# GuyTevet/motion-diffusion-model

Hardware: AMD Instinct MI355X
Metric: motions/sec (B=128, T=196, 50-step DDPM) (higher is better)
Workload: dtype f16x3 (fp32 operands split into fp16 hi+lo, 3 fp16 MFMA products, fp32 accumulate; everything else fp32); 1 GPU; HumanML3D text2motion, 50-step p_sample_loop with CFG 2.5 (2 denoiser forwards per step), batch=128 per GPU, T=196, 8-layer d=512 trans_enc MDM, random-init weights, cached text embedding; global_batch=128, diffusion_steps=50, parallelism=dp1: batch shards, no data-path collective, all_gather of final samples

## Files before the change

motion-diffusion-model_amd/csrc/common.h:

```cpp
#pragma once
#ifdef MDM_EMU
#include "hip_emu.h"
#else
#include <hip/hip_runtime.h>
#define MDM_DYN_SMEM(type, name) \
  extern __shared__ __attribute__((aligned(16))) unsigned char mdm_dyn_smem_raw[]; \
  type* name = reinterpret_cast<type*>(mdm_dyn_smem_raw)
#define MDM_LAUNCH(kernel, grid, block, shmem, stream, ...) \
  hipLaunchKernelGGL(kernel, (grid), (block), (shmem), (stream), __VA_ARGS__)
#endif
#include <stdint.h>
#include <type_traits>
#include <utility>

namespace mdm {

typedef float f32x16 __attribute__((ext_vector_type(16)));
typedef short p16x8 __attribute__((ext_vector_type(8)));

constexpr int kWave = 64;

constexpr int kMaxDevices = 64;
inline int rt_device_ordinal() {
#ifdef MDM_EMU
// ... 231 lines not shown
}

__device__ __forceinline__ void glds16(const void* gsrc_lane, void* lds_wave_base) {
#ifdef MDM_EMU
  emu::vm_issue(static_cast<char*>(lds_wave_base) + 16 * emu::lane_id(), gsrc_lane, 16, false);
#else
  __builtin_amdgcn_global_load_lds((const __attribute__((address_space(1))) void*)gsrc_lane,
                                   (__attribute__((address_space(3))) void*)lds_wave_base, 16, 0, 0);
#endif
}

__device__ __forceinline__ void glds16_nt(const void* gsrc_lane, void* lds_wave_base) {
#ifdef MDM_EMU
  emu::vm_issue(static_cast<char*>(lds_wave_base) + 16 * emu::lane_id(), gsrc_lane, 16, false);
#else
  __builtin_amdgcn_global_load_lds((const __attribute__((address_space(1))) void*)gsrc_lane,
                                   (__attribute__((address_space(3))) void*)lds_wave_base, 16, 0, 2);
#endif
}

template <class F, int... Is>
__device__ __forceinline__ void static_for_impl(F&& f, std::integer_sequence<int, Is...>) {
  (f(std::integral_constant<int, Is>{}), ...);
}
template <int N, class F>
__device__ __forceinline__ void static_for(F&& f) {
  static_for_impl(f, std::make_integer_sequence<int, N>{});
}

#ifdef MDM_EMU
__device__ __forceinline__ void lds_read16(p16x8& dst, const unsigned char* base, uint32_t byte_off) {
  emu::lds_issue(&dst, base + byte_off, 16);
}
template <int N> __device__ __forceinline__ void lds_wait(p16x8&, p16x8&) { emu::lgkm_wait(N); }
template <int N> __device__ __forceinline__ void lds_wait(p16x8&, p16x8&, p16x8&, p16x8&) { emu::lgkm_wait(N); }
template <int N> __device__ __forceinline__ void lds_wait(p16x8&, p16x8&, p16x8&, p16x8&, p16x8&, p16x8&) { emu::lgkm_wait(N); }
template <int N>
__device__ __forceinline__ void lds_wait(p16x8&, p16x8&, p16x8&, p16x8&, p16x8&, p16x8&, p16x8&, p16x8&) { emu::lgkm_wait(N); }
#else
template <int IMM> __device__ __forceinline__ void lds_read16(p16x8& dst, uint32_t lds_addr) {
  asm volatile("ds_read_b128 %0, %1 offset:%2" : "=v"(dst) : "v"(lds_addr), "i"(IMM));
}
template <int N> __device__ __forceinline__ void lds_wait(p16x8& a, p16x8& b) {
  asm volatile("s_waitcnt lgkmcnt(%2)" : "+v"(a), "+v"(b) : "i"(N));
}
template <int N> __device__ __forceinline__ void lds_wait(p16x8& a, p16x8& b, p16x8& c, p16x8& d) {
  asm volatile("s_waitcnt lgkmcnt(%4)" : "+v"(a), "+v"(b), "+v"(c), "+v"(d) : "i"(N));
}
template <int N>
__device__ __forceinline__ void lds_wait(p16x8& a, p16x8& b, p16x8& c, p16x8& d, p16x8& e, p16x8& f, p16x8& g,
                                         p16x8& h) {
  asm volatile("s_waitcnt lgkmcnt(%8)"
               : "+v"(a), "+v"(b), "+v"(c), "+v"(d), "+v"(e), "+v"(f), "+v"(g), "+v"(h)
               : "i"(N));
}
template <int N>
__device__ __forceinline__ void lds_wait(p16x8& a, p16x8& b, p16x8& c, p16x8& d, p16x8& e, p16x8& f) {
  asm volatile("s_waitcnt lgkmcnt(%6)" : "+v"(a), "+v"(b), "+v"(c), "+v"(d), "+v"(e), "+v"(f) : "i"(N));
}
__device__ __forceinline__ uint32_t lds_addr_of(const void* p) {
  return (uint32_t)(uintptr_t)(const __attribute__((address_space(3))) void*)p;
}
#endif

#ifdef MDM_EMU
__device__ __forceinline__ void gload16_async(f32x4& dst, const float* p) { emu::vm_issue(&dst, p, 16, true); }
template <int N> __device__ __forceinline__ void vmem_wait(f32x4&, f32x4&, f32x4&, f32x4&) { emu::vm_wait(N); }
__device__ __forceinline__ void gload16_async(p16x8& dst, const p16_t* p) { emu::vm_issue(&dst, p, 16, true); }
__device__ __forceinline__ void gload16_refill(p16x8& slot, const p16_t* p) { emu::vm_issue(&slot, p, 16, true); }
template <int N> __device__ __forceinline__ void vmem_wait(p16x8&, p16x8&) { emu::vm_wait(N); }
template <int N> __device__ __forceinline__ void vmem_wait(p16x8&, p16x8&, p16x8&, p16x8&) { emu::vm_wait(N); }
template <int N> __device__ __forceinline__ void vmem_wait(p16x8&, p16x8&, p16x8&, p16x8&, p16x8&, p16x8&) { emu::vm_wait(N); }
template <int N>
__device__ __forceinline__ void vmem_wait(p16x8&, p16x8&, p16x8&, p16x8&, p16x8&, p16x8&, p16x8&, p16x8&) { emu::vm_wait(N); }
// ... 197 lines not shown
```

motion-diffusion-model_amd/csrc/gemm_x3.h:

```cpp
#pragma once
#include "attention_x3.h"
#include "common.h"
#include "gemm_f32.h"
#include <cstdlib>

namespace mdm {

constexpr int X3_TM = 224, X3_BK = 32;
constexpr int x3_tn(int waves) { return 32 * waves; }
constexpr int X3_MSUB = X3_TM / 32;
constexpr int X3_A_BYTES = X3_TM * X3_BK * 2;
constexpr int X3_A_STAGE = 2 * X3_A_BYTES;
constexpr int X3_A_RING = 2;
constexpr int X3_PIPE_RING = 4;
#ifndef MDM_X3_EPI_AHEAD
#define MDM_X3_EPI_AHEAD 0
#endif
constexpr bool X3_EPI_AHEAD = MDM_X3_EPI_AHEAD != 0;
#ifdef MDM_X3_PIPE_BADWAIT
constexpr int X3P_MID_SLACK = 8;
#else
constexpr int X3P_MID_SLACK = 0;
#endif
#if defined(MDM_X3_PIPE_WDRAIN)
constexpr int X3P_WAIT_WS = 0, X3P_WAIT_MID = 0;
#elif defined(MDM_X3_PIPE_STRICT)
constexpr int X3P_WAIT_WS = 6, X3P_WAIT_MID = 3;
#else
constexpr int X3P_WAIT_WS = 12, X3P_WAIT_MID = 7;
#endif
constexpr int x3_patch_base(int ring) { return ring * X3_A_STAGE; }
constexpr int X3_PATCH_BYTES = 8 * 32 * 4;
constexpr int X3_TAB_BYTES = X3_TM * 8;
constexpr int x3_tab_base(int waves, int ring = X3_A_RING) { return x3_patch_base(ring) + waves * X3_PATCH_BYTES; }
constexpr int X3_RAW_BYTES = 7 * 1024;
constexpr int x3_raw_base(int waves, int ring = X3_A_RING) { return x3_tab_base(waves, ring) + 2 * X3_TAB_BYTES; }
constexpr int x3_part_base(int waves, int ring = X3_A_RING) { return x3_raw_base(waves, ring) + 2 * X3_RAW_BYTES; }
constexpr int X3_CVEC_BYTES = 4 * 1024;
constexpr int x3_cvec_base(int waves, bool ln, int ring = X3_A_RING) {
  return ln ? x3_part_base(waves, ring) + waves * X3_TAB_BYTES : x3_tab_base(waves, ring);
}
constexpr int x3_lds_bytes(int waves, bool ln, int ring = X3_A_RING) {
  return x3_cvec_base(waves, ln, ring) + 2 * X3_CVEC_BYTES;
}
constexpr int X3_A_GROUPS = X3_A_STAGE / 1024;
constexpr int x3_a_pieces(int waves) { return (X3_A_GROUPS + waves - 1) / waves; }

struct X3Operand {
  const p16_t* hi;
  const p16_t* lo;
};
struct X3Weights {
  const p16_t* hi;
  const p16_t* lo;
};
inline size_t x3_packed_weight_elems(int N, int K) { return (size_t)((N + 31) / 32 * 32) * K; }

struct X3Epilogue {
  float* out;
  const float* bias;
  const float* res;
  const p16_t* resh;
// ... 59 lines not shown
        const float back = p16_to_f32((p16_t)h8[j]);
        bad = bad || !(fabsf(back) <= 3.0e38f);
      }
      if (bad) *overflow = 1;
    }
    const int kstep = k8 >> 1, half = k8 & 1, lane = (n & 31) + 32 * half;
    const size_t o = (((size_t)(n >> 5) * (K / 16) + kstep) * 64 + lane) * 8;
    *reinterpret_cast<p16x8*>(hi + o) = h8;
    *reinterpret_cast<p16x8*>(lo + o) = l8;
  }
}

constexpr int x3_res_rounds(int t, bool t16) { return (t16 && t == X3_MSUB - 1) ? 2 : 4; }
constexpr int x3_res_younger_rounds(int t, int rr, bool t16) {
  int n = 0;
  for (int q = t + 1; q <= t + rr - 1 && q < X3_MSUB; ++q) n += x3_res_rounds(q, t16);
  return n;
}

#if !defined(MDM_EMU) && defined(MDM_PROBES)
#define MDM_X3_DBG 1
__device__ unsigned long long g_x3_dbg[8];
__device__ __forceinline__ unsigned long long x3_now() { return __builtin_readcyclecounter(); }
#endif

template <int PIECES>
struct X3Cursor {
  int v;
  int k;
  uint32_t off[PIECES];
};

template <int WAVES, int ACT, int RES, bool OUT_F32, bool OUT_PLANES, bool OUT_QKV, int ABL, bool FOLD = false,
          bool OSTAT = false, bool EMBED = false, bool T16 = false, bool F6 = false, bool PIPE = false, int NCB = 1>
__global__ __launch_bounds__(64 * WAVES, NCB == 2 ? 1 : 2) void gemm_x3_kernel(X3Operand A, X3Weights W, X3Epilogue ep, int M, int N,
                                                                     int K, int rows_per_tile, int tiles_n, int total) {
  MDM_DYN_SMEM(unsigned char, lds);
  static_assert(!PIPE || (T16 && (WAVES == 8 || (WAVES == 4 && NCB == 2)) && !F6), "the pipelined k-loop exists for 208-row (T16), 256-column tiles");
  static_assert(NCB == 1 || (NCB == 2 && PIPE && WAVES == 4), "two column blocks per wave: the pipelined 4-wave form only");
  constexpr int RINGN = PIPE ? X3_PIPE_RING : X3_A_RING;
  constexpr int NBLK = WAVES * NCB;
  constexpr int X3_WAVES = WAVES, X3_TN = 32 * NBLK, X3_A_PIECES = x3_a_pieces(WAVES);
  constexpr int NT32 = T16 ? X3_MSUB - 1 : X3_MSUB;
  constexpr int NROUNDS = 4 * NT32 + (T16 ? 2 : 0);
  using Cursor = X3Cursor<X3_A_PIECES>;

  const int tid = threadIdx.x;
  const int lane = tid & 63;
#ifdef MDM_EMU
  const int wid = tid >> 6;
#else
  const int wid = __builtin_amdgcn_readfirstlane(tid >> 6);
#endif
  const int r = lane & 31, h = lane >> 5;
  const int nk = K / X3_BK;
  const int gstride = (int)gridDim.x;

  auto tile_origin = [&](int v, int& m0, int& n0) {
    const int lid = xcd_remap(v, total);
    const int tile_m = lid / tiles_n, tile_n = lid - tile_m * tiles_n;
    m0 = tile_m * rows_per_tile;
    n0 = tile_n * X3_TN;
  };

  const int schunk = (lane & 3) ^ ((lane >> 4) & 3);
  auto aim_a = [&](Cursor& c) {
    int m0, n0;
    tile_origin(c.v, m0, n0);
#pragma unroll
    for (int i = 0; i < X3_A_PIECES; ++i) {
      const int jj = min(wid + X3_WAVES * i, 25);
      const int q = PIPE ? (jj < 13 ? jj : jj + 1) : min(wid + X3_WAVES * i, X3_A_GROUPS - 1);
// ... 61 lines not shown
  auto stats_dma = [&](int m0s, int par) {
    const float* st = FOLD ? ep.astat : ep.rstat;
    const int npieces = (X3_TM * ep.stat_parts * 8 + 1023) / 1024;
    for (int pc = wid; pc < npieces; pc += X3_WAVES) {
      const long long total_f = (long long)M * ep.stat_parts * 2;
      long long fo = (long long)m0s * ep.stat_parts * 2 + 4LL * (64 * pc + lane);
      if (fo >= total_f) fo = 0;
      glds16(st + fo, lds + x3_raw_base(NBLK, RINGN) + par * X3_RAW_BYTES + pc * 1024);
    }
  };
  constexpr bool LN_ANY = FOLD || OSTAT || RES == 3;
  auto cvec_dma = [&](int n0c, int par) {
    const float* src = nullptr;
    if (wid == 0) src = ep.bias;
    if constexpr (FOLD) { if (wid == 1) src = ep.colsum; }
    if constexpr (RES == 3) { if (wid == 2) src = ep.rgamma; if (wid == 3) src = ep.rbeta; }
    if (src != nullptr) glds16(src + min(n0c + 4 * lane, N - 4), lds + x3_cvec_base(NBLK, LN_ANY, RINGN) + par * X3_CVEC_BYTES + wid * 1024);
  };
  {
    int m0f, n0f;
    tile_origin(v, m0f, n0f);
    if constexpr (FOLD || RES == 3) stats_dma(m0f, 0);
    cvec_dma(n0f, 0);
  }
  p16x8 wh[2], wl[2], wnh[2], wnl[2];
  p16x8 wsh[4 * NCB] = {}, wsl[4 * NCB] = {};
  uint32_t wso = 0;
  uint32_t wtile = 0;
  auto aim_w_tile = [&]() {
    int m0w, n0w;
    tile_origin(wv, m0w, n0w);
    wtile = (uint32_t)((n0w >> 5) + wid * NCB) * (uint32_t)wk16 * 512u;
  };
  auto aim_w = [&]() { wso = wtile + (uint32_t)wkk * 1024u + (uint32_t)lane * 8u; };
  auto advance_w = [&]() {
    if (++wkk == nk) {
      wkk = 0;
      if (wv + gstride < total) { wv += gstride; aim_w_tile(); }
    }
  };
  auto load_w_half = [&](int ks, auto q_tag) __attribute__((always_inline)) {
    constexpr int q = decltype(q_tag)::value;
#pragma unroll
    for (int cb = 0; cb < NCB; ++cb) {
      const uint32_t o = wso + (uint32_t)cb * (uint32_t)wk16 * 512u + 512u * (uint32_t)ks;
#ifdef MDM_X3_PIPE_NOGUARD
      gload16_async(wsh[q * NCB + cb], W.hi + o);
      gload16_async(wsl[q * NCB + cb], W.lo + o);
#else
      gload16_refill(wsh[q * NCB + cb], W.hi + o);
      gload16_refill(wsl[q * NCB + cb], W.lo + o);
#endif
    }
  };
  auto wait_slot = [&](auto n_tag, auto q_tag) __attribute__((always_inline)) {
    constexpr int n = decltype(n_tag)::value, q = decltype(q_tag)::value;
    if constexpr (NCB == 1) vmem_wait<n>(wsh[q], wsl[q]);
    else vmem_wait<n>(wsh[2 * q], wsl[2 * q], wsh[2 * q + 1], wsl[2 * q + 1]);
  };
  auto wait_all_slots = [&]() __attribute__((always_inline)) {
    static_for<NCB>([&](auto c_tag) __attribute__((always_inline)) {
      constexpr int c4 = 4 * decltype(c_tag)::value;
      vmem_wait<0>(wsh[c4], wsl[c4], wsh[c4 + 1], wsl[c4 + 1], wsh[c4 + 2], wsl[c4 + 2], wsh[c4 + 3], wsl[c4 + 3]);
    });
  };
  int gs = 0;
#if defined(MDM_X3_PIPE_PRIO) && !defined(MDM_EMU)
  if constexpr (PIPE) { if (wid >= 4) __builtin_amdgcn_s_setprio(1); }
#endif
  if constexpr (PIPE) {
#pragma unroll
    for (int st = 0; st < 3; ++st) {
#pragma unroll
      for (int i = 0; i < X3_A_PIECES; ++i) piece_a(ca, i, st);
      advance_a(ca);
    }
    aim_w_tile();
#pragma unroll
    for (int st = 0; st < 2; ++st) {
      aim_w();
      if (st == 0) { load_w_half(0, std::integral_constant<int, 0>{}); load_w_half(1, std::integral_constant<int, 1>{}); }
      else { load_w_half(0, std::integral_constant<int, 2>{}); load_w_half(1, std::integral_constant<int, 3>{}); }
      advance_w();
    }
    wait_all_slots();
    wg_barrier();
  } else {
#pragma unroll
    for (int i = 0; i < X3_A_PIECES; ++i) piece_a(ca, i, 0);
    advance_a(ca);
    load_w(wv, wkk, wh, wl);
    wait_vmem_all();
    wg_barrier();
  }

  int abuf = 0;
  int tile_parity = 0;
  for (; v < total; v += gstride, tile_parity ^= 1) {
    int m0, n0;
    tile_origin(v, m0, n0);
    f32x16 accs_[NCB][NT32];
    f32x4 acc16s_[NCB][2];
#pragma unroll
    for (int cb = 0; cb < NCB; ++cb) {
#pragma unroll
      for (int t = 0; t < NT32; ++t)
#pragma unroll
        for (int e = 0; e < 16; ++e) accs_[cb][t][e] = 0.f;
      acc16s_[cb][0] = f32x4{0.f, 0.f, 0.f, 0.f};
      acc16s_[cb][1] = f32x4{0.f, 0.f, 0.f, 0.f};
    }
    f32x16 (&acc)[NT32] = accs_[0];
    f32x4 (&acc16)[2] = acc16s_[0];
    const int ncol0_w = n0 + wid * NCB * 32;
    const float* const cvec = reinterpret_cast<const float*>(lds + x3_cvec_base(NBLK, LN_ANY, RINGN) + tile_parity * X3_CVEC_BYTES);
    const int kt_cvec = nk > 1 ? 1 : 0;
    if (nk == 1) wg_barrier();
    constexpr bool LN_TABS = FOLD || RES == 3;
    float2* const stab = reinterpret_cast<float2*>(lds + x3_tab_base(NBLK, RINGN) + tile_parity * X3_TAB_BYTES);
    if constexpr (LN_TABS) {
      if (tid < X3_TM) {
        int m0t, n0t;
        tile_origin(v, m0t, n0t);
        const bool pad_row = m0t + tid >= M;
        const float* sraw = reinterpret_cast<const float*>(lds + x3_raw_base(NBLK, RINGN) + tile_parity * X3_RAW_BYTES);
        float s1 = 0.f;
        for (int p = 0; p < ep.stat_parts; ++p) s1 += sraw[(tid * ep.stat_parts + p) * 2];
        const float mean = s1 * ep.inv_dim;
        const float pcols = (float)ep.stat_cols, inv_pcols = 1.0f / pcols;
        float m2 = 0.f;
        for (int p = 0; p < ep.stat_parts; ++p) {
          const float dm = sraw[(tid * ep.stat_parts + p) * 2] * inv_pcols - mean;
          m2 += sraw[(tid * ep.stat_parts + p) * 2 + 1] + pcols * dm * dm;
        }
        const float var = m2 * ep.inv_dim;
#ifdef MDM_EMU
        stab[tid] = pad_row ? make_float2(0.f, 0.f) : make_float2(mean, 1.0f / sqrtf(var + 1e-5f));
#else
        stab[tid] = pad_row ? make_float2(0.f, 0.f) : make_float2(mean, __builtin_amdgcn_rsqf(var + 1e-5f));
#endif
      }
      if (v + gstride < total) {
        int m0n, n0n;
        tile_origin(v + gstride, m0n, n0n);
        stats_dma(m0n, tile_parity ^ 1);
      }
    }
    float2* const atab = stab;
    float2* const rtab = stab;
#ifdef MDM_X3_DBG
    unsigned long long dbg_t0 = 0, dbg_w0 = 0, dbg_w1 = 0, dbg_bar = 0;
    if constexpr ((ABL & 128) != 0) dbg_t0 = x3_now();
#endif
    if constexpr (PIPE) {
#ifndef MDM_X3_PIPE_DEPTH
#define MDM_X3_PIPE_DEPTH 2
#endif
      constexpr int NU = 2 * NT32, NE = NU + 1, XP = NT32, DEPTH = MDM_X3_PIPE_DEPTH, RING = DEPTH + 1;
      constexpr int LWH = 2 * NCB, NA_MIN = 26 / X3_WAVES;
      constexpr int WAIT_WS = (NCB == 1 && X3_WAVES == 8) ? X3P_WAIT_WS : 2 * NA_MIN + 3 * LWH;
      constexpr int WAIT_MID = (NCB == 1 && X3_WAVES == 8) ? X3P_WAIT_MID : NA_MIN + 2 * LWH;
      static_assert((NCB == 1 && X3_WAVES == 8) || (WAIT_WS == 24 && WAIT_MID == 14), "wide form: 4 waves x 2 column blocks");
      static_assert(NU % RING == 0, "fragment ring slots must line up across steps");
      p16x8 ah[RING], al[RING], a16h, a16l;
#ifndef MDM_EMU
      const uint32_t lane_a = lds_base + fa, lane_a16 = lds_base + fa16;
      const uint32_t sw0 = (uint32_t)((h ^ sw) * 16), sw1 = (uint32_t)(((2 + h) ^ sw) * 16);
#endif
      auto issue_reads = [&](auto ee_tag, uint32_t stg) __attribute__((always_inline)) {
        constexpr int ee = decltype(ee_tag)::value;
        if constexpr (ee == XP) {
#ifdef MDM_EMU
          lds_read16(a16h, lds + stg * X3_A_STAGE, fa16);
          lds_read16(a16l, lds + stg * X3_A_STAGE, X3_A_BYTES + fa16);
#else
          lds_read16<0>(a16h, lane_a16 + stg * X3_A_STAGE);
          lds_read16<X3_A_BYTES>(a16l, lane_a16 + stg * X3_A_STAGE);
#endif
        } else {
          constexpr int u = ee < XP ? ee : ee - 1, ks = u / NT32, t = u - ks * NT32;
#ifdef MDM_EMU
          lds_read16(ah[u % RING], lds + stg * X3_A_STAGE, fa + t * 2048 + (((ks * 2 + h) ^ sw) * 16));
          lds_read16(al[u % RING], lds + stg * X3_A_STAGE, X3_A_BYTES + fa + t * 2048 + (((ks * 2 + h) ^ sw) * 16));
#else
          const uint32_t ad = lane_a + stg * X3_A_STAGE + (ks ? sw1 : sw0);
          lds_read16<t * 2048>(ah[u % RING], ad);
          lds_read16<X3_A_BYTES + t * 2048>(al[u % RING], ad);
// ... 275 lines not shown
    constexpr bool COL_SCALE = x3_has_col_scale(ACT, RES);
    const float mult4 = (COL_SCALE && n4 < ep.scale_cols) ? ep.col_scale : 1.f;
    float4 c4 = zero4(), g4 = zero4(), be4 = zero4();
    if constexpr (FOLD) c4 = ld4(cvec + 256 + cl4);
    if constexpr (RES == 3) {
      g4 = ld4(cvec + 512 + cl4);
      be4 = ld4(cvec + 768 + cl4);
    }
    const float bias = cvec[wblk * 32 + r];
    float csum = 0.f;
    if constexpr (FOLD) csum = cvec[256 + wblk * 32 + r];
    const float accs = ep.acc_scale;
    const float4 bb4 = RES == 3 ? make_float4(b4.x + be4.x, b4.y + be4.y, b4.z + be4.z, b4.w + be4.w) : b4;
    auto finish4 = [&](float4 v4, float2 st) __attribute__((always_inline)) {
      v4.x *= accs; v4.y *= accs; v4.z *= accs; v4.w *= accs;
      if constexpr (FOLD) {
        v4.x = st.y * (v4.x - st.x * c4.x) + bb4.x; v4.y = st.y * (v4.y - st.x * c4.y) + bb4.y;
        v4.z = st.y * (v4.z - st.x * c4.z) + bb4.z; v4.w = st.y * (v4.w - st.x * c4.w) + bb4.w;
      } else {
        v4.x += bb4.x; v4.y += bb4.y; v4.z += bb4.z; v4.w += bb4.w;
      }
      if (ACT == ACT_GELU) { v4.x = gelu_erf_fast(v4.x); v4.y = gelu_erf_fast(v4.y); v4.z = gelu_erf_fast(v4.z); v4.w = gelu_erf_fast(v4.w); }
      else if (ACT == ACT_SILU) { v4.x = silu(v4.x); v4.y = silu(v4.y); v4.z = silu(v4.z); v4.w = silu(v4.w); }
      if constexpr (COL_SCALE) { v4.x *= mult4; v4.y *= mult4; v4.z *= mult4; v4.w *= mult4; }
      return v4;
    };
    auto row_stats = [&](auto j_tag) __attribute__((always_inline)) {
      constexpr int j = decltype(j_tag)::value;
      if constexpr (LN_TABS && j < NROUNDS) return stab[(j / 4) * 32 + 8 * (j % 4) + prow];
      else return make_float2(0.f, 1.f);
    };
    auto patch_write = [&](auto j_tag) __attribute__((always_inline)) {
      constexpr int j = decltype(j_tag)::value, t = j / 4, g = j % 4;
      if constexpr (j < 4 * NT32) {
#pragma unroll
        for (int e = 0; e < 4; ++e) patch[((e + 4 * h) << 5) + r] = acc[t][4 * g + e];
      } else if constexpr (T16 && j < NROUNDS) {
        if (h == g) {
#pragma unroll
          for (int cb = 0; cb < 2; ++cb)
#pragma unroll
            for (int e = 0; e < 4; ++e) patch[((e + 4 * (g16 & 1)) << 5) + 16 * cb + r16] = acc16[cb][e];
        }
      }
    };

    if (OUT_QKV) {
      const int Dm = ep.D, SPq = ep.qkv.SP, Hq = ep.qkv.H;
      int ncol_e = ncol0, m0_e = m0;
#ifndef MDM_EMU
      asm volatile("" : "+s"(ncol_e), "+s"(m0_e));
#endif
      const int which = ncol_e / Dm, hcol = ncol_e - which * Dm, head = hcol >> 7, d0 = hcol & 127;
      const size_t shq = (size_t)(m0_e / rows_per_tile) * Hq + head;
      if (ncol0 < N && !(ABL & 1)) {
        if (which == 2) {
          p16_t* vhp = ep.qkv.vh + ((shq * ep.qkv.NKT) * AX_HD + d0 + r) * 32 + 8 * h;
          p16_t* vlp = ep.qkv.vl + ((shq * ep.qkv.NKT) * AX_HD + d0 + r) * 32 + 8 * h;
          const int nkt = ep.qkv.NKT;
#pragma unroll
          for (int t = 0; t < NT32; ++t) {
            if (t < nkt) {
#pragma unroll
              for (int s2 = 0; s2 < 2; ++s2) {
                float vv[8];
#pragma unroll
                for (int j = 0; j < 8; ++j) {
                  if constexpr (FOLD) {
                    const float2 st = atab[32 * t + mfma_row(8 * s2 + j, h)];
                    vv[j] = st.y * (acc[t][8 * s2 + j] * accs - st.x * csum) + bias;
                  } else {
                    vv[j] = acc[t][8 * s2 + j] * accs + bias;
                  }
                }
                p16x8 vh8, vl8;
                split8(vv, vh8, vl8);
                *reinterpret_cast<p16x8*>(vhp + t * (AX_HD * 32) + 16 * s2) = vh8;
                *reinterpret_cast<p16x8*>(vlp + t * (AX_HD * 32) + 16 * s2) = vl8;
              }
            }
          }
          if constexpr (T16) {
            if (NT32 < nkt) {
#pragma unroll
              for (int cb = 0; cb < 2; ++cb) {
                const int cl = 16 * cb + r16;
                const float b16 = lane_bcast(bias, cl);
                const float c16 = FOLD ? lane_bcast(csum, cl) : 0.f;
                float vv[4];
#pragma unroll
                for (int e = 0; e < 4; ++e) {
                  if constexpr (FOLD) {
                    const float2 st = atab[192 + 4 * g16 + e];
                    vv[e] = st.y * (acc16[cb][e] * accs - st.x * c16) + b16;
                  } else {
                    vv[e] = acc16[cb][e] * accs + b16;
                  }
                }
                const size_t o = ((shq * ep.qkv.NKT + NT32) * AX_HD + d0 + cl) * 32 + 4 * ((g16 >> 1) + 2 * (g16 & 1));
                split4_store(ep.qkv.vh + o, ep.qkv.vl + o, make_float4(vv[0], vv[1], vv[2], vv[3]));
              }
            }
          }
        } else {
          p16_t* dh = (which == 0 ? ep.qkv.qh : ep.qkv.kh) + shq * SPq * AX_HD + d0 + pc4;
          p16_t* dl = (which == 0 ? ep.qkv.ql : ep.qkv.kl) + shq * SPq * AX_HD + d0 + pc4;
          const int nkt = ep.qkv.NKT;
          patch_write(std::integral_constant<int, 0>{});
          float2 st_cur = row_stats(std::integral_constant<int, 0>{});
          float4 v_cur = zero4();
          if constexpr (X3_EPI_AHEAD) {
            wave_lds_fence();
            v_cur = ld4(&patch[prow * 32 + pc4]);
            wave_lds_fence();
            patch_write(std::integral_constant<int, 1>{});
          }
          static_for<NROUNDS>([&](auto j_tag) __attribute__((always_inline)) {
            constexpr int j = decltype(j_tag)::value, t = j / 4, g = j % 4;
            float4 v4;
            float2 st_next;
            if constexpr (X3_EPI_AHEAD) {
              wave_lds_fence();
              float4 v_next = zero4();
              if constexpr (j + 1 < NROUNDS) v_next = ld4(&patch[prow * 32 + pc4]);
              st_next = row_stats(std::integral_constant<int, j + 1>{});
              wave_lds_fence();
              patch_write(std::integral_constant<int, j + 2>{});
              v4 = v_cur;
              v_cur = v_next;
            } else {
              wave_lds_fence();
              v4 = ld4(&patch[prow * 32 + pc4]);
              st_next = row_stats(std::integral_constant<int, j + 1>{});
              wave_lds_fence();
              patch_write(std::integral_constant<int, j + 1>{});
// ... 209 lines not shown
  (void)per_cu;
  return 3;
#else
  static int cus_of[kMaxDevices] = {};
  const int dev = rt_device_ordinal();
  int& cus = cus_of[dev];
  if (cus == 0) {
    hipDeviceProp_t prop;
    if (hipGetDeviceProperties(&prop, dev) == hipSuccess) cus = prop.multiProcessorCount;
    if (cus <= 0) cus = 256;
  }
  int wgs = per_cu * cus / 8 * 8;
#ifdef MDM_PROBES
  static const int div = [] { const char* e = getenv("MDM_X3_GRID_DIV"); return e != nullptr && atoi(e) > 1 ? atoi(e) : 1; }();
  wgs = wgs / div / 8 * 8;
#endif
  return wgs > 0 ? wgs : 8;
#endif
}

#ifdef MDM_PROBES
inline int& x3_waves_setting() {
  static int waves = [] {
    const char* e = getenv("MDM_X3_WAVES");
    return (e != nullptr && e[0] == '4') ? 4 : 8;
  }();
  return waves;
}
#else
inline int x3_waves_setting() { return 8; }
#endif

template <int WAVES, int ACT, int RES, bool OUT_F32, bool OUT_PLANES, bool OUT_QKV, int ABL, bool FOLD = false,
          bool OSTAT = false, bool EMBED = false, bool T16 = false, bool F6 = false, bool PIPE = false, int NCB = 1>
inline int launch_gemm_x3_w(const X3Operand& A, const X3Weights& W, const X3Epilogue& ep, int M, int N, int K,
                                int rpt, hipStream_t stream) {
  constexpr int NBLK = WAVES * NCB;
  constexpr int TN = 32 * NBLK;
  constexpr bool LN = FOLD || OSTAT || RES == 3;
  constexpr int RINGN = PIPE ? X3_PIPE_RING : X3_A_RING;
  const int tiles_m = (M + rpt - 1) / rpt, tiles_n = (N + TN - 1) / TN;
  const int total = tiles_m * tiles_n;
  static_assert(!(F6 && T16), "the f16f6 k-loop has no 16-row sub-tile yet");
  auto kfn = &gemm_x3_kernel<WAVES, ACT, RES, OUT_F32, OUT_PLANES, OUT_QKV, ABL, FOLD, OSTAT, EMBED, T16, F6, PIPE, NCB>;
  if (T16 && rpt > X3_TM - 16) return -2;
  if (PIPE && (K / X3_BK) % 2 != 0) return -2;
  if (!x3_has_col_scale(ACT, RES) && ep.scale_cols > 0) return -2;
#ifndef MDM_EMU
  if (x3_lds_bytes(NBLK, LN, RINGN) > 65536) {
    static bool configured[kMaxDevices] = {};
    if (const int rc = rt_dyn_lds_once(kfn, x3_lds_bytes(NBLK, LN, RINGN), configured, stream)) return rc;
  }
#endif
  const int grid = std::min(total, x3_grid_limit((WAVES == 4 && NCB == 1) ? 2 : 1));
  MDM_LAUNCH(kfn, dim3(grid), dim3(64 * WAVES), x3_lds_bytes(NBLK, LN, RINGN), stream, A, W, ep, M, N, K, rpt, tiles_n, total);
  return 0;
}

inline bool x3_wide_setting() {
#ifdef MDM_PROBES
  const char* e = getenv("MDM_X3_WIDE");
  return e != nullptr && e[0] == '1';
#else
  return false;
#endif
}

inline bool x3_pipe_setting(int kind = 0) {
#ifndef MDM_PROBES
  (void)kind;
  return true;
#else
  static const bool on = [] {
    const char* e = getenv("MDM_X3_PIPE");
    return !(e != nullptr && e[0] == '0');
  }();
  static const int kinds = [] {
    const char* e = getenv("MDM_X3_PIPE_KINDS");
    return e != nullptr ? atoi(e) : 0x3f;
  }();
  return on && ((kinds >> kind) & 1);
#endif
}

template <bool T16, bool PIPE = false, bool WIDE = false>
inline int launch_gemm_x3_ln_t(int kind, const X3Operand& A, const X3Weights& W, const X3Epilogue& ep, int M, int N,
                                   int K, int rpt, hipStream_t s) {
#ifdef MDM_PROBES
  if constexpr (WIDE) {
    switch (kind) {
      case 0: return launch_gemm_x3_w<4, ACT_NONE, 0, false, false, true, 0, true, false, false, T16, false, PIPE, 2>(A, W, ep, M, N, K, rpt, s);
      case 1: return launch_gemm_x3_w<4, ACT_NONE, 2, false, true, false, 0, false, true, false, T16, false, PIPE, 2>(A, W, ep, M, N, K, rpt, s);
      case 2: return launch_gemm_x3_w<4, ACT_NONE, 3, false, true, false, 0, false, true, false, T16, false, PIPE, 2>(A, W, ep, M, N, K, rpt, s);
      case 3: return launch_gemm_x3_w<4, ACT_GELU, 0, false, true, false, 0, true, false, false, T16, false, PIPE, 2>(A, W, ep, M, N, K, rpt, s);
      case 4: return launch_gemm_x3_w<4, ACT_NONE, 0, true, false, false, 0, true, false, false, T16, false, PIPE, 2>(A, W, ep, M, N, K, rpt, s);
      default: return -2;
    }
  }
#endif
  switch (kind) {
    case 0: return launch_gemm_x3_w<8, ACT_NONE, 0, false, false, true, 0, true, false, false, T16, false, PIPE>(A, W, ep, M, N, K, rpt, s);
    case 1: return launch_gemm_x3_w<8, ACT_NONE, 2, false, true, false, 0, false, true, false, T16, false, PIPE>(A, W, ep, M, N, K, rpt, s);
    case 2: return launch_gemm_x3_w<8, ACT_NONE, 3, false, true, false, 0, false, true, false, T16, false, PIPE>(A, W, ep, M, N, K, rpt, s);
    case 3: return launch_gemm_x3_w<8, ACT_GELU, 0, false, true, false, 0, true, false, false, T16, false, PIPE>(A, W, ep, M, N, K, rpt, s);
    case 4: return launch_gemm_x3_w<8, ACT_NONE, 0, true, false, false, 0, true, false, false, T16, false, PIPE>(A, W, ep, M, N, K, rpt, s);
    case 5:
      return launch_gemm_x3_w<8, ACT_NONE, 1, false, true, false, 0, false, false, true, T16>(A, W, ep, M, N, K, rpt, s);
    default: return -2;
  }
}
inline bool x3_t16_setting() {
#ifdef MDM_PROBES
  static const bool on = [] {
    const char* e = getenv("MDM_X3_T16");
    return !(e != nullptr && e[0] == '0');
  }();
  return on;
#else
  return true;
#endif
}
inline int launch_gemm_x3_ln(int kind, const X3Operand& A, const X3Weights& W, const X3Epilogue& ep, int M, int N,
                                 int K, int rpt, hipStream_t s) {
  if (rpt <= X3_TM - 16 && x3_t16_setting()) {
    if (kind != 5 && (K / X3_BK) % 2 == 0 && x3_pipe_setting(kind)) {
      if (x3_wide_setting()) return launch_gemm_x3_ln_t<true, true, true>(kind, A, W, ep, M, N, K, rpt, s);
      return launch_gemm_x3_ln_t<true, true>(kind, A, W, ep, M, N, K, rpt, s);
    }
    return launch_gemm_x3_ln_t<true>(kind, A, W, ep, M, N, K, rpt, s);
  }
  return launch_gemm_x3_ln_t<false>(kind, A, W, ep, M, N, K, rpt, s);
}

#ifdef MDM_PROBES
inline int& x3_pipe_probe() { static int on = 0; return on; }
#endif

template <int ACT, int RES, bool OUT_F32, bool OUT_PLANES, bool OUT_QKV, int ABL = 0>
inline int launch_gemm_x3_t(const X3Operand& A, const X3Weights& W, const X3Epilogue& ep, int M, int N, int K,
                                int rpt, hipStream_t stream) {
#ifdef MDM_PROBES
  if (x3_waves_setting() == 4)
    return launch_gemm_x3_w<4, ACT, RES, OUT_F32, OUT_PLANES, OUT_QKV, ABL>(A, W, ep, M, N, K, rpt, stream);
#endif
  return launch_gemm_x3_w<8, ACT, RES, OUT_F32, OUT_PLANES, OUT_QKV, ABL>(A, W, ep, M, N, K, rpt, stream);
}

inline int launch_gemm_x3(const X3Operand& A, const X3Weights& W, const X3Epilogue& ep, int M, int N, int K, int act,
                              int seq_len, hipStream_t s, int ablate = 0) {
  const bool res = ep.res != nullptr, f32 = ep.out != nullptr, pl = ep.oh != nullptr;
  const int rpt = x3_rows_per_tile(M, seq_len);
  if (ep.resh != nullptr) {
    if (ablate == 0 && act == ACT_NONE && !res && f32 && !pl)
      return launch_gemm_x3_t<ACT_NONE, 2, true, false, false>(A, W, ep, M, N, K, rpt, s);
    return -2;
  }
#ifdef MDM_PROBES
  if (x3_pipe_probe() != 0 && act == ACT_NONE && !res && f32 && !pl && M % 197 == 0 && (K / X3_BK) % 2 == 0) {
#define X3_PIPE_PROBE_CASE(c) case c: return x3_pipe_probe() == 1 \
      ? launch_gemm_x3_w<8, ACT_NONE, 0, true, false, false, c, false, false, false, true, false, true>(A, W, ep, M, N, K, 197, s) \
// ... 33 lines not shown
  if (act == ACT_NONE && res && f32 && !pl) return launch_gemm_x3_t<ACT_NONE, 1, true, false, false>(A, W, ep, M, N, K, rpt, s);
  if (act == ACT_GELU && !res && !f32 && pl) return launch_gemm_x3_t<ACT_GELU, 0, false, true, false>(A, W, ep, M, N, K, rpt, s);
  if (act == ACT_GELU && !res && f32 && !pl) return launch_gemm_x3_t<ACT_GELU, 0, true, false, false>(A, W, ep, M, N, K, rpt, s);
  if (act == ACT_GELU && res && f32 && !pl) return launch_gemm_x3_t<ACT_GELU, 1, true, false, false>(A, W, ep, M, N, K, rpt, s);
  if (act == ACT_SILU && !res && f32 && !pl) return launch_gemm_x3_t<ACT_SILU, 0, true, false, false>(A, W, ep, M, N, K, rpt, s);
  return -2;
}

#ifdef MDM_PROBES
inline int launch_gemm_f16f6(const X3Operand& A, const X3Weights& W, const X3Epilogue& ep, int M, int N, int K, int act,
                             hipStream_t s) {
  const bool res = ep.res != nullptr;
  if (act == ACT_NONE && !res && x3_waves_setting() == 4)
    return launch_gemm_x3_w<4, ACT_NONE, 0, true, false, false, 0, false, false, false, false, true>(A, W, ep, M, N, K, X3_TM, s);
  if (act == ACT_NONE && !res)
    return launch_gemm_x3_w<8, ACT_NONE, 0, true, false, false, 0, false, false, false, false, true>(A, W, ep, M, N, K, X3_TM, s);
  if (act == ACT_NONE && res)
    return launch_gemm_x3_w<8, ACT_NONE, 1, true, false, false, 0, false, false, false, false, true>(A, W, ep, M, N, K, X3_TM, s);
  if (act == ACT_GELU && !res)
    return launch_gemm_x3_w<8, ACT_GELU, 0, true, false, false, 0, false, false, false, false, true>(A, W, ep, M, N, K, X3_TM, s);
  return -2;
}
#endif

inline int launch_gemm_x3_qkv(const X3Operand& A, const X3Weights& W, const X3Epilogue& ep, int nseq, int S, int D,
                                  hipStream_t s) {
  if (S > X3_TM) return -2;
  if (x3_waves_setting() == 8 && S <= X3_TM - 16 && x3_t16_setting()) {
    if ((D / X3_BK) % 2 == 0 && x3_pipe_setting(5)) {
#ifdef MDM_PROBES
      if (x3_wide_setting())
        return launch_gemm_x3_w<4, ACT_NONE, 0, false, false, true, 0, false, false, false, true, false, true, 2>(A, W, ep, nseq * S,
                                                                                                                   3 * D, D, S, s);
#endif
      return launch_gemm_x3_w<8, ACT_NONE, 0, false, false, true, 0, false, false, false, true, false, true>(A, W, ep, nseq * S,
                                                                                                              3 * D, D, S, s);
    }
    return launch_gemm_x3_w<8, ACT_NONE, 0, false, false, true, 0, false, false, false, true>(A, W, ep, nseq * S, 3 * D, D,
                                                                                                 S, s);
  }
  return launch_gemm_x3_t<ACT_NONE, 0, false, false, true>(A, W, ep, nseq * S, 3 * D, D, S, s);
}

#endif

}
```

Measured before the change: 365.4 motions/s.

## Use 16x16x32 MFMA tiling in the pipelined x3 GEMM k-loop

Measured after the change: 396.3 motions/s (median of 6 runs). +8.5%, better.

```diff
diff --git a/motion-diffusion-model_amd/csrc/common.h b/motion-diffusion-model_amd/csrc/common.h
--- a/motion-diffusion-model_amd/csrc/common.h
+++ b/motion-diffusion-model_amd/csrc/common.h
@@ -287,6 +287,9 @@
 __device__ __forceinline__ void lds_read16(p16x8& dst, const unsigned char* base, uint32_t byte_off) {
   emu::lds_issue(&dst, base + byte_off, 16);
 }
+__device__ __forceinline__ void lds_refill16(p16x8& slot, const unsigned char* base, uint32_t byte_off) {
+  emu::lds_issue(&slot, base + byte_off, 16);
+}
 template <int N> __device__ __forceinline__ void lds_wait(p16x8&, p16x8&) { emu::lgkm_wait(N); }
 template <int N> __device__ __forceinline__ void lds_wait(p16x8&, p16x8&, p16x8&, p16x8&) { emu::lgkm_wait(N); }
 template <int N> __device__ __forceinline__ void lds_wait(p16x8&, p16x8&, p16x8&, p16x8&, p16x8&, p16x8&) { emu::lgkm_wait(N); }
@@ -295,6 +298,9 @@
 #else
 template <int IMM> __device__ __forceinline__ void lds_read16(p16x8& dst, uint32_t lds_addr) {
   asm volatile("ds_read_b128 %0, %1 offset:%2" : "=v"(dst) : "v"(lds_addr), "i"(IMM));
+}
+template <int IMM> __device__ __forceinline__ void lds_refill16(p16x8& slot, uint32_t lds_addr) {
+  asm volatile("ds_read_b128 %0, %1 offset:%2" : "+v"(slot) : "v"(lds_addr), "i"(IMM));
 }
 template <int N> __device__ __forceinline__ void lds_wait(p16x8& a, p16x8& b) {
   asm volatile("s_waitcnt lgkmcnt(%2)" : "+v"(a), "+v"(b) : "i"(N));
diff --git a/motion-diffusion-model_amd/csrc/gemm_x3.h b/motion-diffusion-model_amd/csrc/gemm_x3.h
--- a/motion-diffusion-model_amd/csrc/gemm_x3.h
+++ b/motion-diffusion-model_amd/csrc/gemm_x3.h
@@ -28,6 +28,13 @@
 constexpr int X3P_WAIT_WS = 6, X3P_WAIT_MID = 3;
 #else
 constexpr int X3P_WAIT_WS = 12, X3P_WAIT_MID = 7;
+#endif
+#if defined(MDM_X3_PIPE_WDRAIN)
+constexpr int X3M_WAIT_WS = 0, X3M_WAIT_MID = 0;
+#elif defined(MDM_X3_PIPE_STRICT)
+constexpr int X3M_WAIT_WS = 4, X3M_WAIT_MID = 3;
+#else
+constexpr int X3M_WAIT_WS = 7, X3M_WAIT_MID = 11;
 #endif
 constexpr int x3_patch_base(int ring) { return ring * X3_A_STAGE; }
 constexpr int X3_PATCH_BYTES = 8 * 32 * 4;
@@ -153,12 +160,14 @@
 };
 
 template <int WAVES, int ACT, int RES, bool OUT_F32, bool OUT_PLANES, bool OUT_QKV, int ABL, bool FOLD = false,
-          bool OSTAT = false, bool EMBED = false, bool T16 = false, bool F6 = false, bool PIPE = false, int NCB = 1>
+          bool OSTAT = false, bool EMBED = false, bool T16 = false, bool F6 = false, bool PIPE = false, int NCB = 1,
+          bool M16 = false>
 __global__ __launch_bounds__(64 * WAVES, NCB == 2 ? 1 : 2) void gemm_x3_kernel(X3Operand A, X3Weights W, X3Epilogue ep, int M, int N,
                                                                      int K, int rows_per_tile, int tiles_n, int total) {
   MDM_DYN_SMEM(unsigned char, lds);
   static_assert(!PIPE || (T16 && (WAVES == 8 || (WAVES == 4 && NCB == 2)) && !F6), "the pipelined k-loop exists for 208-row (T16), 256-column tiles");
   static_assert(NCB == 1 || (NCB == 2 && PIPE && WAVES == 4), "two column blocks per wave: the pipelined 4-wave form only");
+  static_assert(!M16 || (PIPE && WAVES == 8 && NCB == 1 && ABL == 0), "the 16x16x32 form: pipelined, 8 waves, no ablations");
   constexpr int RINGN = PIPE ? X3_PIPE_RING : X3_A_RING;
   constexpr int NBLK = WAVES * NCB;
   constexpr int X3_WAVES = WAVES, X3_TN = 32 * NBLK, X3_A_PIECES = x3_a_pieces(WAVES);
@@ -286,7 +295,9 @@
     tile_origin(wv, m0w, n0w);
     wtile = (uint32_t)((n0w >> 5) + wid * NCB) * (uint32_t)wk16 * 512u;
   };
-  auto aim_w = [&]() { wso = wtile + (uint32_t)wkk * 1024u + (uint32_t)lane * 8u; };
+  const uint32_t lane_wo = M16 ? (uint32_t)((lane >> 5) * 512 + ((lane & 15) + 32 * ((lane >> 4) & 1)) * 8) : (uint32_t)lane * 8u;
+  constexpr uint32_t W_HALF = M16 ? 128u : 512u;
+  auto aim_w = [&]() { wso = wtile + (uint32_t)wkk * 1024u + lane_wo; };
   auto advance_w = [&]() {
     if (++wkk == nk) {
       wkk = 0;
@@ -297,7 +308,7 @@
     constexpr int q = decltype(q_tag)::value;
 #pragma unroll
     for (int cb = 0; cb < NCB; ++cb) {
-      const uint32_t o = wso + (uint32_t)cb * (uint32_t)wk16 * 512u + 512u * (uint32_t)ks;
+      const uint32_t o = wso + (uint32_t)cb * (uint32_t)wk16 * 512u + W_HALF * (uint32_t)ks;
 #ifdef MDM_X3_PIPE_NOGUARD
       gload16_async(wsh[q * NCB + cb], W.hi + o);
       gload16_async(wsl[q * NCB + cb], W.lo + o);
@@ -355,14 +366,21 @@
     tile_origin(v, m0, n0);
     f32x16 accs_[NCB][NT32];
     f32x4 acc16s_[NCB][2];
-#pragma unroll
-    for (int cb = 0; cb < NCB; ++cb) {
-#pragma unroll
-      for (int t = 0; t < NT32; ++t)
-#pragma unroll
-        for (int e = 0; e < 16; ++e) accs_[cb][t][e] = 0.f;
-      acc16s_[cb][0] = f32x4{0.f, 0.f, 0.f, 0.f};
-      acc16s_[cb][1] = f32x4{0.f, 0.f, 0.f, 0.f};
+    constexpr int NS16 = 2 * X3_MSUB - 1;
+    f32x4 accm_[M16 ? NS16 : 1][2];
+    if constexpr (M16) {
+#pragma unroll
+      for (int s = 0; s < NS16; ++s) accm_[s][0] = accm_[s][1] = f32x4{0.f, 0.f, 0.f, 0.f};
+    } else {
+#pragma unroll
+      for (int cb = 0; cb < NCB; ++cb) {
+#pragma unroll
+        for (int t = 0; t < NT32; ++t)
+#pragma unroll
+          for (int e = 0; e < 16; ++e) accs_[cb][t][e] = 0.f;
+        acc16s_[cb][0] = f32x4{0.f, 0.f, 0.f, 0.f};
+        acc16s_[cb][1] = f32x4{0.f, 0.f, 0.f, 0.f};
+      }
     }
     f32x16 (&acc)[NT32] = accs_[0];
     f32x4 (&acc16)[2] = acc16s_[0];
@@ -406,7 +424,79 @@
     unsigned long long dbg_t0 = 0, dbg_w0 = 0, dbg_w1 = 0, dbg_bar = 0;
     if constexpr ((ABL & 128) != 0) dbg_t0 = x3_now();
 #endif
-    if constexpr (PIPE) {
+    if constexpr (M16) {
+      constexpr int NE = NS16, DEPTH = 2, RING = DEPTH + 1, XB = NE / 2;
+      auto slot = [](int e) constexpr { return e == NE - 1 ? RING : e % RING; };
+      p16x8 ah[RING + 1] = {}, al[RING + 1] = {};
+#ifndef MDM_EMU
+      const uint32_t lane_a = lds_base + fa16 - 192 * 64;
+#endif
+      auto issue_reads = [&](auto e_tag, uint32_t stg) __attribute__((always_inline)) {
+        constexpr int e = decltype(e_tag)::value;
+#ifdef MDM_EMU
+        lds_refill16(ah[slot(e)], lds + stg * X3_A_STAGE, fa16 - 192 * 64 + e * 1024);
+        lds_refill16(al[slot(e)], lds + stg * X3_A_STAGE, X3_A_BYTES + fa16 - 192 * 64 + e * 1024);
+#else
+        lds_refill16<e * 1024>(ah[slot(e)], lane_a + stg * X3_A_STAGE);
+        lds_refill16<X3_A_BYTES + e * 1024>(al[slot(e)], lane_a + stg * X3_A_STAGE);
+#endif
+      };
+      auto pipe_step = [&](auto par_tag) __attribute__((always_inline)) {
+        constexpr int PAR = decltype(par_tag)::value, W0 = 2 * PAR, W1 = 2 * PAR + 1;
+        const uint32_t cur = (uint32_t)gs & 3u, nxt = (uint32_t)(gs + 1) & 3u, fill = (uint32_t)(gs + 3) & 3u;
+        vmem_wait<X3M_WAIT_WS>(wsh[W0], wsl[W0], wsh[W1], wsl[W1]);
+        static_for<NE>([&](auto e_tag) __attribute__((always_inline)) {
+          constexpr int e = decltype(e_tag)::value;
+          if constexpr (e + DEPTH < NE) issue_reads(std::integral_constant<int, e + DEPTH>{}, cur);
+          else issue_reads(std::integral_constant<int, e + DEPTH - NE>{}, nxt);
+          if constexpr (e == XB) {
+            vmem_wait<X3M_WAIT_MID + X3P_MID_SLACK>(wsh[W0], wsl[W0], wsh[W1], wsl[W1]);
+#ifndef MDM_EMU
+            __builtin_amdgcn_sched_barrier(0);
+#endif
+            wg_barrier_nodrain();
+#ifndef MDM_EMU
+            __builtin_amdgcn_sched_barrier(0);
+#endif
+          }
+          lds_wait<2 * DEPTH>(ah[slot(e)], al[slot(e)]);
+#ifndef MDM_EMU
+          __builtin_amdgcn_sched_barrier(0);
+#endif
+#pragma unroll
+          for (int c = 0; c < 2; ++c) accm_[e][c] = mfma16_p16(al[slot(e)], wsh[W0 + c], accm_[e][c]);
+#pragma unroll
+          for (int c = 0; c < 2; ++c) accm_[e][c] = mfma16_p16(ah[slot(e)], wsl[W0 + c], accm_[e][c]);
+#pragma unroll
+          for (int c = 0; c < 2; ++c) accm_[e][c] = mfma16_p16(ah[slot(e)], wsh[W0 + c], accm_[e][c]);
+#ifndef MDM_EMU
+          __builtin_amdgcn_sched_barrier(0);
+#endif
+          if constexpr (e >= XB && e < XB + X3_A_PIECES) piece_a(ca, e - XB, (int)fill);
+#ifndef MDM_EMU
+          __builtin_amdgcn_sched_barrier(0);
+#endif
+        });
+        aim_w();
+        load_w_half(0, std::integral_constant<int, W0>{});
+        load_w_half(1, std::integral_constant<int, W1>{});
+        advance_w();
+        advance_a(ca);
+        ++gs;
+      };
+      static_for<DEPTH>([&](auto d_tag) __attribute__((always_inline)) { issue_reads(d_tag, (uint32_t)gs & 3u); });
+      for (int kt = 0; kt < nk; kt += 2) {
+        pipe_step(std::integral_constant<int, 0>{});
+        if (kt == 0 && v + gstride < total) {
+          int m0n, n0n;
+          tile_origin(v + gstride, m0n, n0n);
+          cvec_dma(n0n, tile_parity ^ 1);
+        }
+        pipe_step(std::integral_constant<int, 1>{});
+      }
+      lds_wait<0>(ah[0], al[0], ah[1], al[1]);
+      wait_all_slots();
+    } else if constexpr (PIPE) {
 #ifndef MDM_X3_PIPE_DEPTH
 #define MDM_X3_PIPE_DEPTH 2
 #endif
@@ -748,7 +838,16 @@
     };
     auto patch_write = [&](auto j_tag) __attribute__((always_inline)) {
       constexpr int j = decltype(j_tag)::value, t = j / 4, g = j % 4;
-      if constexpr (j < 4 * NT32) {
+      if constexpr (M16) {
+        if constexpr (j < NROUNDS) {
+          if (h == j % 2) {
+#pragma unroll
+            for (int cb = 0; cb < 2; ++cb)
+#pragma unroll
+              for (int e = 0; e < 4; ++e) patch[((e + 4 * (g16 & 1)) << 5) + 16 * cb + r16] = accm_[j / 2][cb][e];
+          }
+        }
+      } else if constexpr (j < 4 * NT32) {
 #pragma unroll
         for (int e = 0; e < 4; ++e) patch[((e + 4 * h) << 5) + r] = acc[t][4 * g + e];
       } else if constexpr (T16 && j < NROUNDS) {
@@ -774,6 +873,32 @@
           p16_t* vhp = ep.qkv.vh + ((shq * ep.qkv.NKT) * AX_HD + d0 + r) * 32 + 8 * h;
           p16_t* vlp = ep.qkv.vl + ((shq * ep.qkv.NKT) * AX_HD + d0 + r) * 32 + 8 * h;
           const int nkt = ep.qkv.NKT;
+          if constexpr (M16) {
+#pragma unroll
+            for (int cb = 0; cb < 2; ++cb) {
+              const int cl = 16 * cb + r16;
+              const float b16 = cvec[wblk * 32 + cl];
+              const float c16 = FOLD ? cvec[256 + wblk * 32 + cl] : 0.f;
+              const size_t o0 = (shq * ep.qkv.NKT * AX_HD + d0 + cl) * 32 + 4 * ((g16 >> 1) + 2 * (g16 & 1));
+#pragma unroll
+              for (int s = 0; s < NS16; ++s) {
+                if ((s >> 1) < nkt) {
+                  float vv[4];
+#pragma unroll
+                  for (int e = 0; e < 4; ++e) {
+                    if constexpr (FOLD) {
+                      const float2 st = atab[16 * s + 4 * g16 + e];
+                      vv[e] = st.y * (accm_[s][cb][e] * accs - st.x * c16) + b16;
+                    } else {
+                      vv[e] = accm_[s][cb][e] * accs + b16;
+                    }
+                  }
+                  const size_t o = o0 + (size_t)(s >> 1) * (AX_HD * 32) + 16 * (s & 1);
+                  split4_store(ep.qkv.vh + o, ep.qkv.vl + o, make_float4(vv[0], vv[1], vv[2], vv[3]));
+                }
+              }
+            }
+          } else {
 #pragma unroll
           for (int t = 0; t < NT32; ++t) {
             if (t < nkt) {
@@ -817,6 +942,7 @@
                 split4_store(ep.qkv.vh + o, ep.qkv.vl + o, make_float4(vv[0], vv[1], vv[2], vv[3]));
               }
             }
+          }
           }
         } else {
           p16_t* dh = (which == 0 ? ep.qkv.qh : ep.qkv.kh) + shq * SPq * AX_HD + d0 + pc4;
@@ -1092,7 +1218,8 @@
 #endif
 
 template <int WAVES, int ACT, int RES, bool OUT_F32, bool OUT_PLANES, bool OUT_QKV, int ABL, bool FOLD = false,
-          bool OSTAT = false, bool EMBED = false, bool T16 = false, bool F6 = false, bool PIPE = false, int NCB = 1>
+          bool OSTAT = false, bool EMBED = false, bool T16 = false, bool F6 = false, bool PIPE = false, int NCB = 1,
+          bool M16 = false>
 inline int launch_gemm_x3_w(const X3Operand& A, const X3Weights& W, const X3Epilogue& ep, int M, int N, int K,
                                 int rpt, hipStream_t stream) {
   constexpr int NBLK = WAVES * NCB;
@@ -1102,7 +1229,7 @@
   const int tiles_m = (M + rpt - 1) / rpt, tiles_n = (N + TN - 1) / TN;
   const int total = tiles_m * tiles_n;
   static_assert(!(F6 && T16), "the f16f6 k-loop has no 16-row sub-tile yet");
-  auto kfn = &gemm_x3_kernel<WAVES, ACT, RES, OUT_F32, OUT_PLANES, OUT_QKV, ABL, FOLD, OSTAT, EMBED, T16, F6, PIPE, NCB>;
+  auto kfn = &gemm_x3_kernel<WAVES, ACT, RES, OUT_F32, OUT_PLANES, OUT_QKV, ABL, FOLD, OSTAT, EMBED, T16, F6, PIPE, NCB, M16>;
   if (T16 && rpt > X3_TM - 16) return -2;
   if (PIPE && (K / X3_BK) % 2 != 0) return -2;
   if (!x3_has_col_scale(ACT, RES) && ep.scale_cols > 0) return -2;
@@ -1143,7 +1270,7 @@
 #endif
 }
 
-template <bool T16, bool PIPE = false, bool WIDE = false>
+template <bool T16, bool PIPE = false, bool WIDE = false, bool M16 = false>
 inline int launch_gemm_x3_ln_t(int kind, const X3Operand& A, const X3Weights& W, const X3Epilogue& ep, int M, int N,
                                    int K, int rpt, hipStream_t s) {
 #ifdef MDM_PROBES
@@ -1159,12 +1286,13 @@
   }
 #endif
   switch (kind) {
-    case 0: return launch_gemm_x3_w<8, ACT_NONE, 0, false, false, true, 0, true, false, false, T16, false, PIPE>(A, W, ep, M, N, K, rpt, s);
-    case 1: return launch_gemm_x3_w<8, ACT_NONE, 2, false, true, false, 0, false, true, false, T16, false, PIPE>(A, W, ep, M, N, K, rpt, s);
-    case 2: return launch_gemm_x3_w<8, ACT_NONE, 3, false, true, false, 0, false, true, false, T16, false, PIPE>(A, W, ep, M, N, K, rpt, s);
-    case 3: return launch_gemm_x3_w<8, ACT_GELU, 0, false, true, false, 0, true, false, false, T16, false, PIPE>(A, W, ep, M, N, K, rpt, s);
-    case 4: return launch_gemm_x3_w<8, ACT_NONE, 0, true, false, false, 0, true, false, false, T16, false, PIPE>(A, W, ep, M, N, K, rpt, s);
+    case 0: return launch_gemm_x3_w<8, ACT_NONE, 0, false, false, true, 0, true, false, false, T16, false, PIPE, 1, M16>(A, W, ep, M, N, K, rpt, s);
+    case 1: return launch_gemm_x3_w<8, ACT_NONE, 2, false, true, false, 0, false, true, false, T16, false, PIPE, 1, M16>(A, W, ep, M, N, K, rpt, s);
+    case 2: return launch_gemm_x3_w<8, ACT_NONE, 3, false, true, false, 0, false, true, false, T16, false, PIPE, 1, M16>(A, W, ep, M, N, K, rpt, s);
+    case 3: return launch_gemm_x3_w<8, ACT_GELU, 0, false, true, false, 0, true, false, false, T16, false, PIPE, 1, M16>(A, W, ep, M, N, K, rpt, s);
+    case 4: return launch_gemm_x3_w<8, ACT_NONE, 0, true, false, false, 0, true, false, false, T16, false, PIPE, 1, M16>(A, W, ep, M, N, K, rpt, s);
     case 5:
+      if constexpr (M16) return -2;
       return launch_gemm_x3_w<8, ACT_NONE, 1, false, true, false, 0, false, false, true, T16>(A, W, ep, M, N, K, rpt, s);
     default: return -2;
   }
@@ -1180,12 +1308,26 @@
   return true;
 #endif
 }
+inline bool x3_m16_setting() {
+#ifdef MDM_PROBES
+  static const bool on = [] {
+    const char* e = getenv("MDM_X3_M32");
+    return !(e != nullptr && e[0] == '1');
+  }();
+  return on;
+#else
+  return true;
+#endif
+}
 inline int launch_gemm_x3_ln(int kind, const X3Operand& A, const X3Weights& W, const X3Epilogue& ep, int M, int N,
                                  int K, int rpt, hipStream_t s) {
   if (rpt <= X3_TM - 16 && x3_t16_setting()) {
     if (kind != 5 && (K / X3_BK) % 2 == 0 && x3_pipe_setting(kind)) {
+#ifdef MDM_PROBES
       if (x3_wide_setting()) return launch_gemm_x3_ln_t<true, true, true>(kind, A, W, ep, M, N, K, rpt, s);
-      return launch_gemm_x3_ln_t<true, true>(kind, A, W, ep, M, N, K, rpt, s);
+      if (!x3_m16_setting()) return launch_gemm_x3_ln_t<true, true>(kind, A, W, ep, M, N, K, rpt, s);
+#endif
+      return launch_gemm_x3_ln_t<true, true, false, true>(kind, A, W, ep, M, N, K, rpt, s);
     }
     return launch_gemm_x3_ln_t<true>(kind, A, W, ep, M, N, K, rpt, s);
   }
@@ -1285,9 +1427,12 @@
       if (x3_wide_setting())
         return launch_gemm_x3_w<4, ACT_NONE, 0, false, false, true, 0, false, false, false, true, false, true, 2>(A, W, ep, nseq * S,
                                                                                                                    3 * D, D, S, s);
-#endif
-      return launch_gemm_x3_w<8, ACT_NONE, 0, false, false, true, 0, false, false, false, true, false, true>(A, W, ep, nseq * S,
-                                                                                                              3 * D, D, S, s);
+      if (!x3_m16_setting())
+        return launch_gemm_x3_w<8, ACT_NONE, 0, false, false, true, 0, false, false, false, true, false, true>(A, W, ep, nseq * S,
+                                                                                                                3 * D, D, S, s);
+#endif
+      return launch_gemm_x3_w<8, ACT_NONE, 0, false, false, true, 0, false, false, false, true, false, true, 1, true>(
+          A, W, ep, nseq * S, 3 * D, D, S, s);
     }
     return launch_gemm_x3_w<8, ACT_NONE, 0, false, false, true, 0, false, false, false, true>(A, W, ep, nseq * S, 3 * D, D,
                                                                                                  S, s);
```
